# kai422/DAS3R

Hardware: AMD Instinct MI355X
Metric: render fwd+bwd Msplats/s at 1080p (higher is better)
Workload: dtype f32; 1 GPU; 1M random splats, 1920x1080, SH degree 3, forward+backward (BASELINE.json configs[3], constant P); splats_per_gpu=1000000, splats_per_gpu_final=1000000, init_steps=30, sh_degree=3, num_rendered=2614506, api=GaussianRasterizer.forward + autograd backward (drop-in surface), parallelism=1 independent scenes, one per GPU

## Files before the change

das3r_amd/csrc/preprocess.hip:

```cpp
#include "common.h"
#include "granule.h"
#include "segkey.h"
#include "splat_math.h"
#include "pretransform_math.h"

namespace das3r {

template <bool HAS_SH, bool HAS_COV, bool STAGE, bool AA = false>
__global__ void __launch_bounds__(256) preprocess_kernel(
    int P, int D, int M, const float *__restrict__ means3D, const float *__restrict__ scales, float scale_modifier,
    const float *__restrict__ rotations, const float *__restrict__ opacities, const float *__restrict__ shs,
    const float *__restrict__ cov3D_precomp, const float *__restrict__ colors_precomp, const float *__restrict__ viewmatrix,
    const float *__restrict__ projmatrix, const float *__restrict__ campos, int W, int H, float tanfovx, float tanfovy,
    int tiles_x, int tiles_y, int32_t *__restrict__ radii, uint32_t *__restrict__ depth_key, float4 *__restrict__ xyh,
    float4 *__restrict__ conic_opacity, float4 *__restrict__ rgbd, uint8_t *__restrict__ clamped,
    uint32_t *__restrict__ tiles_touched, uint32_t *__restrict__ rect32, int tight_rect , uint32_t *__restrict__ zero_a, uint32_t zero_a_words, uint32_t *__restrict__ zero_b,
    uint32_t zero_b_words, uint32_t *__restrict__ zero_c, uint32_t zero_c_words, unsigned long long *__restrict__ arrive,
    uint32_t *__restrict__ host_out, uint32_t tag, const EmitArgs em,
    uint32_t *__restrict__ dhist ,
    uint32_t dhist_mask ,
    uint32_t *__restrict__ dhist_next ,
    const PreXform pre ,
    float *__restrict__ shjac ) {
    const int gidx = blockIdx.x * blockDim.x + threadIdx.x;
    bool sampled = false;
    if (dhist != nullptr) {
        uint32_t h = blockIdx.x * 0x9E3779B1u;
        h ^= h >> 15; h *= 0x85EBCA6Bu; h ^= h >> 13; h *= 0xC2B2AE35u; h ^= h >> 16;
        sampled = (h & dhist_mask) == 0u;
    }
    const bool live = gidx < P;
    const int idx = live ? gidx : P - 1;
    float3 p, s_in = make_float3(0.f, 0.f, 0.f);
    float op;
    float4 q_in = make_float4(0.f, 0.f, 0.f, 0.f);
    float c3_in[6] = {0.f, 0.f, 0.f, 0.f, 0.f, 0.f};
    if (!HAS_COV && pre.xyz != nullptr) {
        PoseRegs pose;
        load_pose(pre.Rm, pre.tv, pre.Lq, pose);
        const float rx = pre.xyz[3 * idx], ry = pre.xyz[3 * idx + 1], rz = pre.xyz[3 * idx + 2];
        const float4 rq = reinterpret_cast<const float4 *>(pre.rot)[idx];
        const float r0 = pre.scaling[3 * idx], r1 = pre.scaling[3 * idx + 1], r2 = pre.scaling[3 * idx + 2];
        const float ro = pre.opacity_raw[idx];
        const float rc = pre.conf_flat[pre.mask_index ? pre.mask_index[idx] : (int64_t)idx];
        p = pre_mean(pose, rx, ry, rz);
        q_in = pre_rot(pose, rq);
        s_in = make_float3(pre_scale(r0), pre_scale(r1), pre_scale(r2));
        op = pre_opacity(ro, rc);
    } else {
        p = make_float3(means3D[3 * idx], means3D[3 * idx + 1], means3D[3 * idx + 2]);
        op = opacities[idx];
        if (HAS_COV) {
#pragma unroll
            for (int i = 0; i < 6; i++) c3_in[i] = cov3D_precomp[6 * idx + i];
        } else {
            s_in = make_float3(scales[3 * idx], scales[3 * idx + 1], scales[3 * idx + 2]);
            q_in = reinterpret_cast<const float4 *>(rotations)[idx];
        }
    }
    __shared__ uint32_t s_tiles;
    if (threadIdx.x == 0) s_tiles = 0;
    if (!STAGE) __syncthreads();
    for (uint32_t i = gidx; i < zero_a_words; i += gridDim.x * blockDim.x) zero_a[i] = 0u;
    for (uint32_t i = gidx; i < zero_b_words; i += gridDim.x * blockDim.x) zero_b[i] = 0u;
    for (uint32_t i = gidx; i < zero_c_words; i += gridDim.x * blockDim.x) zero_c[i] = 0u;
    if (dhist_next != nullptr && gidx < DBINS) dhist_next[gidx] = 0u;
    __shared__ float4 sh_lds[STAGE ? 256 * 13 : 256 * 5];
    if (STAGE) {
        const float4 *src = reinterpret_cast<const float4 *>(shs) + (size_t)blockIdx.x * 256 * 12;
        const size_t limit = (size_t)P * 12 - (size_t)blockIdx.x * 256 * 12;
        float4 v[12];
#pragma unroll
        for (int i = 0; i < 12; i++) {
            const size_t f = (size_t)(i * 256 + threadIdx.x);
            v[i] = src[f < limit ? f : limit - 1];
        }
#pragma unroll
        for (int i = 0; i < 12; i++) {
            const int f = i * 256 + threadIdx.x;
            sh_lds[(f / 12) * 13 + (f % 12)] = v[i];
        }
        __syncthreads();
    }
    float V[16], PM[16];
#pragma unroll
    for (int i = 0; i < 16; i++) {
        V[i] = viewmatrix[i];
        PM[i] = projmatrix[i];
    }
    const float focal_x = W / (2.0f * tanfovx), focal_y = H / (2.0f * tanfovy);

    int radius_out = 0;
    uint32_t key_out = 0xFFFFFFFFu, tiles_out = 0;
    uint8_t clamp_out = 0;
    float4 xy_out = make_float4(0.f, 0.f, -1e30f, -1e30f);
    float4 co_out = make_float4(0.f, 0.f, 0.f, 0.f);
    float4 rgbd_out = make_float4(0.f, 0.f, 0.f, 0.f);
    float jac_out[9] = {0.f, 0.f, 0.f, 0.f, 0.f, 0.f, 0.f, 0.f, 0.f};
    int bx0 = 0, by0 = 0, bx1 = 0, by1 = 0;

    const float3 p_view = xform43(p, V);
    if (p_view.z > NEAR_PLANE) {
        const float4 p_hom = xform44(p, PM);
        const float p_w = 1.0f / (p_hom.w + 0.0000001f);
        const float ndc_x = p_hom.x * p_w, ndc_y = p_hom.y * p_w;

        float c3[6];
        if (HAS_COV) {
#pragma unroll
            for (int i = 0; i < 6; i++) c3[i] = c3_in[i];
        } else {
            cov3d_from_scale_rot(s_in, scale_modifier, q_in, c3);
        }
        float T[2][3];
        float3 t;
        bool cx, cy;
        ewa_T(p_view, V, focal_x, focal_y, tanfovx, tanfovy, T, t, cx, cy);
        float a, b, c, a0 = 0.f, c0 = 0.f;
        if constexpr (AA) {
            cov2d_undilated(T, c3, a0, b, c0);
            a = a0 + 0.3f;
            c = c0 + 0.3f;
        } else {
            cov2d_from_T(T, c3, a, b, c);
        }
        const float det = a * c - b * b;
        if (det != 0.0f) {
            const float det_inv = 1.f / det;
            const float conA = c * det_inv, conB = -b * det_inv, conC = a * det_inv;
            const float mid = 0.5f * (a + c);
            const float lambda1 = mid + sqrtf(fmaxf(0.1f, mid * mid - det));
            const float lambda2 = mid - sqrtf(fmaxf(0.1f, mid * mid - det));
            const float my_radius = ceilf(3.f * sqrtf(fmaxf(lambda1, lambda2)));
            const float px = ((ndc_x + 1.0f) * W - 1.0f) * 0.5f;
            const float py = ((ndc_y + 1.0f) * H - 1.0f) * 0.5f;
            const int r = (int)my_radius;
            int rminx, rminy, rmaxx, rmaxy;
            tile_rect(px, py, r, tiles_x, tiles_y, rminx, rminy, rmaxx, rmaxy);
            const int area = (rmaxx - rminx) * (rmaxy - rminy);
            if (area != 0) {
                float3 col;
                if (HAS_SH && STAGE) {
                    float sh[48];
                    const int n4 = (3 * (D + 1) * (D + 1) + 3) >> 2;
#pragma unroll
                    for (int i = 0; i < 12; i++) {
                        if (i < n4) {
                            const float4 v = sh_lds[threadIdx.x * 13 + i];
                            sh[4 * i] = v.x; sh[4 * i + 1] = v.y; sh[4 * i + 2] = v.z; sh[4 * i + 3] = v.w;
                        }
                    }
                    col = sh_regs_to_rgb(D, sh, p, campos, clamp_out);
                    if (shjac != nullptr) sh_ddir_regs(D, sh, p, campos, jac_out);
                } else if (HAS_SH) {
                    float sh[48];
                    const float *row = shs + (size_t)idx * M * 3;
                    load_sh_row(row, D, sh_vec_ok(row, D, M), sh);
                    col = sh_regs_to_rgb(D, sh, p, campos, clamp_out);
                    if (shjac != nullptr) sh_ddir_regs(D, sh, p, campos, jac_out);
                } else {
                    col = make_float3(colors_precomp[3 * idx], colors_precomp[3 * idx + 1], colors_precomp[3 * idx + 2]);
                }
                radius_out = r;
                key_out = __float_as_uint(p_view.z);
                if constexpr (AA) op = op * aa_factor(aa_rho(a0, b, c0, det));
                float hx = -1e30f, hy = -1e30f;
                if (255.0f * op > 1.0f) {
                    const float tau2 = 2.0f * __logf(255.0f * op) * 1.0005f + 1e-3f;
                    hx = sqrtf(tau2 * a) * 1.0005f + 0.02f;
                    hy = sqrtf(tau2 * c) * 1.0005f + 0.02f;
                }
                xy_out = make_float4(px, py, hx, hy);
                binned_rect(xy_out, r, tiles_x, tiles_y, (tight_rect & 1) != 0, bx0, by0, bx1, by1);
                tiles_out = (uint32_t)((bx1 - bx0) * (by1 - by0));
                co_out = make_float4(conA, conB, conC, op);
                rgbd_out = make_float4(col.x, col.y, col.z, p_view.z);
            }
        }
    } else if ((tight_rect & 2) && live) {
        __hip_atomic_store(host_out + 12, tag, __ATOMIC_RELAXED, __HIP_MEMORY_SCOPE_SYSTEM);
        __threadfence_system();
    }
    if (live) {
    radii[idx] = radius_out;
    depth_key[idx] = key_out;
    tiles_touched[idx] = tiles_out;
    rect32[idx] = tiles_out ? ((uint32_t)bx0 | ((uint32_t)bx1 << 8) | ((uint32_t)by0 << 16) | ((uint32_t)by1 << 24)) : 0u;
    clamped[idx] = clamp_out;
    if (HAS_SH && shjac != nullptr) {
#pragma unroll
        for (int j = 0; j < 9; j++) shjac[(size_t)j * P + idx] = jac_out[j];
    }
    }
    {
        __syncthreads();
        float4 *rec = sh_lds;
        const int t = threadIdx.x, slot = t * 5;
        rec[slot] = xy_out;
        rec[slot + 1] = co_out;
        rec[slot + 2] = rgbd_out;
        rec[slot + 3] = make_float4(__int_as_float(radius_out), __uint_as_float(tiles_out), 0.f, 0.f);
        __syncthreads();
        float4 *dst = xyh + (size_t)blockIdx.x * 256 * SPLAT_REC;
        const size_t lim = ((size_t)P - (size_t)blockIdx.x * 256) * SPLAT_REC;
#pragma unroll
        for (int i = 0; i < 4; i++) {
            const int f = i * 256 + t;
            if ((size_t)f < lim) dst[f] = rec[f + (f >> 2)];
        }
        if (em.status != nullptr || sampled) __syncthreads();
    }
    if (sampled) {
        uint32_t *lh = reinterpret_cast<uint32_t *>(sh_lds);
        lh[threadIdx.x] = 0u;
        __syncthreads();
        if (live && tiles_out) atomicAdd(&lh[depth_bin(key_out)], tiles_out);
        __syncthreads();
        const uint32_t c = lh[threadIdx.x];
        if (c) atomicAdd(&dhist[threadIdx.x], c);
    }

    if (em.status != nullptr) {
        __shared__ uint32_t ws[4], s_carry;
        uint32_t(*h)[RADIX_SIZE] = reinterpret_cast<uint32_t(*)[RADIX_SIZE]>(sh_lds);
        const int tid = threadIdx.x, lane = __lane_id(), wave = tid >> 6;
        const uint32_t b = blockIdx.x;
        const uint32_t mine = live ? tiles_out : 0u;
        uint32_t total;
        const uint32_t ex = block_exclusive_scan_256(mine, ws, &total);
#pragma unroll
        for (int q = 0; q < 4; q++) h[q][tid] = 0u;
        if (wave == 0) {
            constexpr uint32_t GS = 64u;
            const uint32_t grp = b / GS, r = b % GS, nblocks = gridDim.x;
            const u64 t64 = (u64)em.tag << 32;
            if (lane == 0) granule_store(em.status + b, t64 | total);
            uint32_t in_group = 0, before = 0;
            unsigned spins = 0;
            {
                const bool has = (uint32_t)lane < r;
                u64 x = t64;
                while (true) {
                    if (has) x = granule_poll(em.status + (b - r) + lane, spins);
                    if (__all((x >> 32) == (u64)em.tag)) break;
                    if (spins == SOFT_SPINS && lane == 0) atomicOr(em.err, ERR_HARD_POLL);
                    if (++spins > SPIN_LIMIT) { if (lane == 0) atomicOr(em.err, ERR_TIMEOUT); break; }
                    __builtin_amdgcn_s_sleep(2);
                }
                in_group = has ? (uint32_t)x : 0u;
#pragma unroll
                for (int o = 32; o >= 1; o >>= 1) in_group += (uint32_t)__shfl_xor((int)in_group, o, 64);
            }
            if (r == GS - 1u && lane == 0) granule_store(em.status + nblocks + grp, t64 | (u64)(in_group + total));
            for (uint32_t p0 = 0; p0 < grp; p0 += 64u) {
                const bool has = p0 + (uint32_t)lane < grp;
                u64 x = t64;
                while (true) {
                    if (has) x = granule_poll(em.status + nblocks + p0 + lane, spins);
                    if (__all((x >> 32) == (u64)em.tag)) break;
                    if (spins == SOFT_SPINS && lane == 0) atomicOr(em.err, ERR_HARD_POLL);
                    if (++spins > SPIN_LIMIT) { if (lane == 0) atomicOr(em.err, ERR_TIMEOUT); break; }
                    __builtin_amdgcn_s_sleep(2);
                }
                uint32_t v = has ? (uint32_t)x : 0u;
#pragma unroll
                for (int o = 32; o >= 1; o >>= 1) v += (uint32_t)__shfl_xor((int)v, o, 64);
                before += v;
            }
            if (lane == 0) s_carry = in_group + before;
        }
        __syncthreads();
        uint32_t o = s_carry + ex;
        if (live) {
            em.off_by_gid[idx] = o;
            for (int y = by0; y < by1; y++)
                for (int x = bx0; x < bx1; x++) {
                    if (o < em.cap) {
                        const uint32_t t = (uint32_t)(y * tiles_x + x);
                        em.tile_keys[o] = t;
                        em.gids[o] = (uint32_t)idx;
                        for (int q = 0, sh = 0, dw = tile_digit_width(em.tbits); sh < em.tbits; q++, sh += dw) {
                            const int bits = (em.tbits - sh) < dw ? (em.tbits - sh) : dw;
                            atomicAdd(&h[q][(t >> sh) & ((1u << bits) - 1u)], 1u);
                        }
                    }
                    o++;
                }
        }
        if (b == gridDim.x - 1 && tid == 0) {
            const uint32_t count = s_carry + total, flags = *em.err;
            em.count[0] = count;
            em.count[1] = flags;
            em.count_out[0] = count;
            em.count_out[1] = flags;
            __hip_atomic_store(em.count_out + 2, em.tag, __ATOMIC_RELEASE, __HIP_MEMORY_SCOPE_SYSTEM);
        }
        __syncthreads();
        for (int q = 0, sh = 0, dw = tile_digit_width(em.tbits); sh < em.tbits; q++, sh += dw) {
            const uint32_t c = h[q][tid];
            if (c) atomicAdd(&em.ghist[q * RADIX_SIZE + tid], c);
        }
        return;
    }
    if (arrive == nullptr) return;
    uint32_t wsum = live ? tiles_out : 0u;
#pragma unroll
    for (int o = 32; o >= 1; o >>= 1) wsum += (uint32_t)__shfl_xor((int)wsum, o, 64);
    if (__lane_id() == 0 && wsum) atomicAdd(&s_tiles, wsum);
    __syncthreads();
    if (threadIdx.x == 0) {
        constexpr unsigned long long LOW = (1ull << 40) - 1ull;
        const unsigned r = blockIdx.x & 63u;
        const unsigned long long expected = (gridDim.x - r + 63u) / 64u;
        unsigned long long mine = (1ull << 40) | (unsigned long long)s_tiles;
        unsigned long long *sub = arrive + 8 + 8 * r;
        unsigned long long old = atomicAdd(sub, mine);
        if ((old >> 40) + 1ull == expected) {
            __hip_atomic_store(sub, 0ull, __ATOMIC_RELAXED, __HIP_MEMORY_SCOPE_AGENT);
            mine = (1ull << 40) | ((old + mine) & LOW);
            old = atomicAdd(arrive, mine);
            const unsigned long long subs = gridDim.x < 64u ? gridDim.x : 64u;
            if ((old >> 40) + 1ull == subs) {
                const unsigned long long total = (old + mine) & LOW;
                __hip_atomic_store(arrive, 0ull, __ATOMIC_RELAXED, __HIP_MEMORY_SCOPE_AGENT);
                host_out[0] = (uint32_t)(total > 0xFFFFFFFFull ? 0xFFFFFFFFull : total);
                __hip_atomic_store(host_out + 2, tag, __ATOMIC_RELEASE, __HIP_MEMORY_SCOPE_SYSTEM);
            }
        }
    }
}

__global__ void __launch_bounds__(256) mark_visible_kernel(int P, const float *__restrict__ means3D,
                                                           const float *__restrict__ viewmatrix, uint8_t *__restrict__ present) {
    const int idx = blockIdx.x * blockDim.x + threadIdx.x;
    if (idx >= P) return;
    float V[16];
#pragma unroll
    for (int i = 0; i < 16; i++) V[i] = viewmatrix[i];
    const float3 p = make_float3(means3D[3 * idx], means3D[3 * idx + 1], means3D[3 * idx + 2]);
    present[idx] = xform43(p, V).z > NEAR_PLANE ? 1 : 0;
}

int launch_preprocess(const das3r_raster_args *a, const das3r_raster_in *in, int32_t *radii, char *geom, char *img, char *binning_ctrl,
                      size_t binning_ctrl_bytes, const Layout &L, unsigned long long *arrive, uint32_t *host_out, uint32_t tag,
                      hipStream_t s, const EmitArgs *emit, uint32_t *dhist, uint32_t *dhist_next, bool aa) {
    const int P = a->P;
    if (P == 0) return DAS3R_OK;
    const EmitArgs em = emit ? *emit : EmitArgs{nullptr, 0u, nullptr, nullptr, nullptr, nullptr, nullptr, 0u, 0, nullptr, nullptr};
    dim3 grid(div_up(P, 256)), block(256);
    uint32_t dhist_mask = 0u;
    while ((grid.x >> __builtin_popcount(dhist_mask)) > 512u) dhist_mask = (dhist_mask << 1) | 1u;
    const bool has_sh = in->shs != nullptr, has_cov = in->cov3D_precomp != nullptr;
    const PreXform pre = pre_xform(in);
    float *const shjac = has_sh && L.g_shjac ? (float *)(geom + L.g_shjac) : nullptr;
#define ARGS                                                                                                              \
    P, a->sh_degree, a->M, in->means3D, in->scales, a->scale_modifier, in->rotations, in->opacities, in->shs,             \
        in->cov3D_precomp, in->colors_precomp, a->viewmatrix, a->projmatrix, a->campos, a->image_width, a->image_height,  \
        a->tanfovx, a->tanfovy, L.tiles_x, L.tiles_y, radii, (uint32_t *)(geom + L.g_keyA), (float4 *)(geom + L.pub.xy),  \
        (float4 *)(geom + L.pub.conic_opacity), (float4 *)(geom + L.pub.rgbd), (uint8_t *)(geom + L.pub.clamped),         \
        (uint32_t *)(geom + L.pub.tiles_touched), (uint32_t *)(geom + L.g_rect), (use_tight_rect() ? 1 : 0) | (a->prefiltered ? 2 : 0), (uint32_t *)(geom + L.g_ghist), (uint32_t)(L.g_ctrl_bytes / 4),                 \
        (uint32_t *)(img + L.pub.ranges), (uint32_t)(2 * L.ntiles), (uint32_t *)binning_ctrl, (uint32_t)(binning_ctrl_bytes / 4), arrive, host_out, tag, em, dhist, dhist_mask, dhist_next, pre, shjac
    const bool stage = has_sh && a->M == 16 && a->sh_degree >= 2 && ((uintptr_t)in->shs & 15) == 0 && !switches().no_sh_stage;
#define LAUNCH_PRE(SH, COV, ST)                                                                                   \
    do {                                                                                                          \
        if (aa) DAS3R_LAUNCH((preprocess_kernel<SH, COV, ST, true>), grid, block, 0, s, ARGS);                   \
        else DAS3R_LAUNCH((preprocess_kernel<SH, COV, ST>), grid, block, 0, s, ARGS);                            \
    } while (0)
    if (has_sh && !has_cov && stage) LAUNCH_PRE(true, false, true);
    else if (has_sh && has_cov && stage) LAUNCH_PRE(true, true, true);
    else if (has_sh && !has_cov) LAUNCH_PRE(true, false, false);
    else if (has_sh && has_cov) LAUNCH_PRE(true, true, false);
    else if (!has_sh && !has_cov) LAUNCH_PRE(false, false, false);
    else LAUNCH_PRE(false, true, false);
#undef LAUNCH_PRE
#undef ARGS
    KERNEL_CHECK(s, a->debug, "preprocess");
    return DAS3R_OK;
}

int launch_mark_visible(int P, const float *means3D, const float *viewmatrix, uint8_t *present, hipStream_t s) {
    if (P == 0) return DAS3R_OK;
    DAS3R_LAUNCH(mark_visible_kernel, dim3(div_up(P, 256)), dim3(256), 0, s, P, means3D, viewmatrix, present);
    KERNEL_CHECK(s, false, "mark_visible");
    return DAS3R_OK;
}

}
```

das3r_amd/csrc/splat_math.h:

```cpp
#pragma once
#include <hip/hip_runtime.h>

namespace das3r {

__device__ constexpr float SH_C0 = 0.28209479177387814f;
__device__ constexpr float SH_C1 = 0.4886025119029199f;
__device__ constexpr float SH_C2_0 = 1.0925484305920792f, SH_C2_1 = -1.0925484305920792f, SH_C2_2 = 0.31539156525252005f,
                           SH_C2_3 = -1.0925484305920792f, SH_C2_4 = 0.5462742152960396f;
__device__ constexpr float SH_C3_0 = -0.5900435899266435f, SH_C3_1 = 2.890611442640554f, SH_C3_2 = -0.4570457994644658f,
                           SH_C3_3 = 0.3731763325901154f, SH_C3_4 = -0.4570457994644658f, SH_C3_5 = 1.445305721320277f,
                           SH_C3_6 = -0.5900435899266435f;

__device__ __forceinline__ float3 xform43(const float3 p, const float *m) {
    return make_float3(m[0] * p.x + m[4] * p.y + m[8] * p.z + m[12], m[1] * p.x + m[5] * p.y + m[9] * p.z + m[13],
                       m[2] * p.x + m[6] * p.y + m[10] * p.z + m[14]);
}
__device__ __forceinline__ float4 xform44(const float3 p, const float *m) {
    return make_float4(m[0] * p.x + m[4] * p.y + m[8] * p.z + m[12], m[1] * p.x + m[5] * p.y + m[9] * p.z + m[13],
                       m[2] * p.x + m[6] * p.y + m[10] * p.z + m[14], m[3] * p.x + m[7] * p.y + m[11] * p.z + m[15]);
}

__device__ __forceinline__ void quat_to_R(const float4 q, float R[3][3]) {
    const float r = q.x, x = q.y, y = q.z, z = q.w;
    R[0][0] = 1.f - 2.f * (y * y + z * z); R[0][1] = 2.f * (x * y - r * z);       R[0][2] = 2.f * (x * z + r * y);
    R[1][0] = 2.f * (x * y + r * z);       R[1][1] = 1.f - 2.f * (x * x + z * z); R[1][2] = 2.f * (y * z - r * x);
    R[2][0] = 2.f * (x * z - r * y);       R[2][1] = 2.f * (y * z + r * x);       R[2][2] = 1.f - 2.f * (x * x + y * y);
}

__device__ __forceinline__ void cov3d_from_scale_rot(const float3 scale, const float mod, const float4 q, float *cov) {
    float R[3][3];
    quat_to_R(q, R);
    const float s[3] = {mod * scale.x, mod * scale.y, mod * scale.z};
    float Mm[3][3];
#pragma unroll
    for (int i = 0; i < 3; i++)
#pragma unroll
        for (int k = 0; k < 3; k++) Mm[i][k] = R[i][k] * s[k];
#define SIG(i, j) (Mm[i][0] * Mm[j][0] + Mm[i][1] * Mm[j][1] + Mm[i][2] * Mm[j][2])
    cov[0] = SIG(0, 0); cov[1] = SIG(0, 1); cov[2] = SIG(0, 2); cov[3] = SIG(1, 1); cov[4] = SIG(1, 2); cov[5] = SIG(2, 2);
#undef SIG
}

__device__ __forceinline__ void ewa_T(const float3 p_view, const float *V, const float focal_x, const float focal_y,
                                      const float tanfovx, const float tanfovy, float T[2][3], float3 &t, bool &clampx, bool &clampy) {
    t = p_view;
    const float limx = 1.3f * tanfovx, limy = 1.3f * tanfovy;
    const float txtz = t.x / t.z, tytz = t.y / t.z;
    clampx = (txtz < -limx || txtz > limx);
    clampy = (tytz < -limy || tytz > limy);
    t.x = fminf(limx, fmaxf(-limx, txtz)) * t.z;
    t.y = fminf(limy, fmaxf(-limy, tytz)) * t.z;
    const float J00 = focal_x / t.z, J02 = -(focal_x * t.x) / (t.z * t.z);
    const float J11 = focal_y / t.z, J12 = -(focal_y * t.y) / (t.z * t.z);
#pragma unroll
    for (int j = 0; j < 3; j++) {
        T[0][j] = J00 * V[4 * j + 0] + 0.f * V[4 * j + 1] + J02 * V[4 * j + 2];
        T[1][j] = 0.f * V[4 * j + 0] + J11 * V[4 * j + 1] + J12 * V[4 * j + 2];
    }
}

__device__ __forceinline__ void cov2d_undilated(const float T[2][3], const float *c3, float &a0, float &b, float &c0) {
    const float S[3][3] = {{c3[0], c3[1], c3[2]}, {c3[1], c3[3], c3[4]}, {c3[2], c3[4], c3[5]}};
    float TS[2][3];
#pragma unroll
    for (int i = 0; i < 2; i++)
#pragma unroll
        for (int j = 0; j < 3; j++) TS[i][j] = T[i][0] * S[0][j] + T[i][1] * S[1][j] + T[i][2] * S[2][j];
    a0 = TS[0][0] * T[0][0] + TS[0][1] * T[0][1] + TS[0][2] * T[0][2];
    b = TS[0][0] * T[1][0] + TS[0][1] * T[1][1] + TS[0][2] * T[1][2];
    c0 = TS[1][0] * T[1][0] + TS[1][1] * T[1][1] + TS[1][2] * T[1][2];
}

__device__ __forceinline__ void cov2d_from_T(const float T[2][3], const float *c3, float &a, float &b, float &c) {
    float a0, c0;
    cov2d_undilated(T, c3, a0, b, c0);
    a = a0 + 0.3f;
    c = c0 + 0.3f;
}

constexpr float AA_RHO_MIN = 2.5e-5f;
__device__ __forceinline__ float aa_rho(const float a0, const float b, const float c0, const float det) { return (a0 * c0 - b * b) / det; }
__device__ __forceinline__ float aa_factor(const float rho) { return sqrtf(fmaxf(rho, AA_RHO_MIN)); }

__device__ __forceinline__ void tile_rect(const float px, const float py, const int r, const int tiles_x, const int tiles_y,
                                          int &rminx, int &rminy, int &rmaxx, int &rmaxy) {
    rminx = min(tiles_x, max(0, (int)((px - r) / TILE_X)));
    rminy = min(tiles_y, max(0, (int)((py - r) / TILE_Y)));
    rmaxx = min(tiles_x, max(0, (int)((px + r + TILE_X - 1) / TILE_X)));
    rmaxy = min(tiles_y, max(0, (int)((py + r + TILE_Y - 1) / TILE_Y)));
}

__device__ __forceinline__ void binned_rect(const float4 xyh, const int r, const int tiles_x, const int tiles_y, const bool tight,
                                            int &rminx, int &rminy, int &rmaxx, int &rmaxy) {
    tile_rect(xyh.x, xyh.y, r, tiles_x, tiles_y, rminx, rminy, rmaxx, rmaxy);
    if (tight) {
        if (xyh.z < 0.f) {
            rmaxx = rminx;
            return;
        }
        const float px0 = ceilf(xyh.x - xyh.z), px1 = floorf(xyh.x + xyh.z);
        const float py0 = ceilf(xyh.y - xyh.w), py1 = floorf(xyh.y + xyh.w);
        if (px1 < px0 || py1 < py0 || px1 < 0.f || py1 < 0.f) {
            rmaxx = rminx;
            return;
        }
        const int tx0 = (int)fmaxf(px0, 0.f) >> 4, ty0 = (int)fmaxf(py0, 0.f) >> 4;
        const int tx1 = ((int)fminf(px1, 1.0e6f) >> 4) + 1, ty1 = ((int)fminf(py1, 1.0e6f) >> 4) + 1;
        rminx = max(rminx, tx0);
        rminy = max(rminy, ty0);
        rmaxx = max(rminx, min(rmaxx, tx1));
        rmaxy = max(rminy, min(rmaxy, ty1));
    }
}

__device__ __forceinline__ void load_sh_row(const float *__restrict__ row, const int D, const bool vec_ok, float sh[48]) {
    const int n3 = 3 * (D + 1) * (D + 1);
    if (vec_ok) {
        const float4 *r4 = reinterpret_cast<const float4 *>(row);
#pragma unroll
        for (int i = 0; i < 12; i++) {
            if (4 * i < n3) {
                const float4 v = r4[i];
                sh[4 * i] = v.x; sh[4 * i + 1] = v.y; sh[4 * i + 2] = v.z; sh[4 * i + 3] = v.w;
            }
        }
    } else {
#pragma unroll
        for (int i = 0; i < 48; i++)
            if (i < n3) sh[i] = row[i];
    }
}

__device__ __forceinline__ float3 sh_eval(const int deg, const float sh[48], const float x, const float y, const float z) {
    float out[3];
#pragma unroll
    for (int c = 0; c < 3; c++) {
#define SHC(k) sh[(k) * 3 + c]
        float r = SH_C0 * SHC(0);
        if (deg > 0) {
            r = r - SH_C1 * y * SHC(1) + SH_C1 * z * SHC(2) - SH_C1 * x * SHC(3);
            if (deg > 1) {
                const float xx = x * x, yy = y * y, zz = z * z, xy = x * y, yz = y * z, xz = x * z;
                r = r + SH_C2_0 * xy * SHC(4) + SH_C2_1 * yz * SHC(5) + SH_C2_2 * (2.f * zz - xx - yy) * SHC(6) +
                    SH_C2_3 * xz * SHC(7) + SH_C2_4 * (xx - yy) * SHC(8);
                if (deg > 2) {
                    r = r + SH_C3_0 * y * (3.f * xx - yy) * SHC(9) + SH_C3_1 * xy * z * SHC(10) +
                        SH_C3_2 * y * (4.f * zz - xx - yy) * SHC(11) + SH_C3_3 * z * (2.f * zz - 3.f * xx - 3.f * yy) * SHC(12) +
                        SH_C3_4 * x * (4.f * zz - xx - yy) * SHC(13) + SH_C3_5 * z * (xx - yy) * SHC(14) +
                        SH_C3_6 * x * (xx - 3.f * yy) * SHC(15);
                }
            }
        }
#undef SHC
        out[c] = r + 0.5f;
    }
    return make_float3(out[0], out[1], out[2]);
}

#define SH_DDIR(SHC, dRdx, dRdy, dRdz)                                                                                          \
    do {                                                                                                                        \
        dRdx = 0.f; dRdy = 0.f; dRdz = 0.f;                                                                                     \
        if (D > 0) {                                                                                                            \
            dRdx = -SH_C1 * SHC(3);                                                                                             \
            dRdy = -SH_C1 * SHC(1);                                                                                             \
            dRdz = SH_C1 * SHC(2);                                                                                              \
            if (D > 1) {                                                                                                        \
                dRdx += SH_C2_0 * y * SHC(4) + SH_C2_2 * 2.f * -x * SHC(6) + SH_C2_3 * z * SHC(7) + SH_C2_4 * 2.f * x * SHC(8); \
                dRdy += SH_C2_0 * x * SHC(4) + SH_C2_1 * z * SHC(5) + SH_C2_2 * 2.f * -y * SHC(6) + SH_C2_4 * 2.f * -y * SHC(8); \
                dRdz += SH_C2_1 * y * SHC(5) + SH_C2_2 * 2.f * 2.f * z * SHC(6) + SH_C2_3 * x * SHC(7);                       \
                if (D > 2) {                                                                                                    \
                    dRdx += SH_C3_0 * SHC(9) * 3.f * 2.f * xy + SH_C3_1 * SHC(10) * yz + SH_C3_2 * SHC(11) * -2.f * xy +       \
                            SH_C3_3 * SHC(12) * -3.f * 2.f * xz + SH_C3_4 * SHC(13) * (-3.f * xx + 4.f * zz - yy) +            \
                            SH_C3_5 * SHC(14) * 2.f * xz + SH_C3_6 * SHC(15) * 3.f * (xx - yy);                                \
                    dRdy += SH_C3_0 * SHC(9) * 3.f * (xx - yy) + SH_C3_1 * SHC(10) * xz +                                      \
                            SH_C3_2 * SHC(11) * (-3.f * yy + 4.f * zz - xx) + SH_C3_3 * SHC(12) * -3.f * 2.f * yz +            \
                            SH_C3_4 * SHC(13) * -2.f * xy + SH_C3_5 * SHC(14) * -2.f * yz + SH_C3_6 * SHC(15) * -3.f * 2.f * xy; \
                    dRdz += SH_C3_1 * SHC(10) * xy + SH_C3_2 * SHC(11) * 4.f * 2.f * yz +                                      \
                            SH_C3_3 * SHC(12) * 3.f * (2.f * zz - xx - yy) + SH_C3_4 * SHC(13) * 4.f * 2.f * xz +              \
                            SH_C3_5 * SHC(14) * (xx - yy);                                                                      \
                }                                                                                                               \
            }                                                                                                                   \
        }                                                                                                                       \
    } while (0)

__device__ __forceinline__ bool sh_vec_ok(const float *row, const int D, const int M) {
    const int n3 = 3 * (D + 1) * (D + 1);
    return (((uintptr_t)row & 15) == 0) && (((n3 + 3) & ~3) <= 3 * M);
}

__device__ __forceinline__ float3 sh_regs_to_rgb(const int D, const float sh[48], const float3 p, const float *campos,
                                                 uint8_t &clamp_bits) {
    const float dx = p.x - campos[0], dy = p.y - campos[1], dz = p.z - campos[2];
    const float inv = 1.f / sqrtf(dx * dx + dy * dy + dz * dz);
    const float3 r = sh_eval(D, sh, dx * inv, dy * inv, dz * inv);
    clamp_bits = (uint8_t)((r.x < 0.f ? 1 : 0) | (r.y < 0.f ? 2 : 0) | (r.z < 0.f ? 4 : 0));
    return make_float3(fmaxf(r.x, 0.f), fmaxf(r.y, 0.f), fmaxf(r.z, 0.f));
}

__device__ __forceinline__ void sh_ddir_regs(const int D, const float sh[48], const float3 p, const float *campos, float J[9]) {
    const float dx = p.x - campos[0], dy = p.y - campos[1], dz = p.z - campos[2];
    const float inv = 1.f / sqrtf(dx * dx + dy * dy + dz * dz);
    const float x = dx * inv, y = dy * inv, z = dz * inv;
    const float xx = x * x, yy = y * y, zz = z * z, xy = x * y, yz = y * z, xz = x * z;
#pragma unroll
    for (int c = 0; c < 3; c++) {
#define SHC_REG(k) sh[(k) * 3 + c]
        SH_DDIR(SHC_REG, J[3 * c], J[3 * c + 1], J[3 * c + 2]);
#undef SHC_REG
    }
}

}
```

Measured before the change: 1143 Msplats/s.

## Split SH staging into two LDS phases to shrink shared memory and raise occupancy

The staged preprocess kernel now stages spherical-harmonic coefficients through shared memory in two halves: the first 7 float4s per splat are evaluated first, then the remaining 5 are written into the same LDS buffer and evaluated. This cuts LDS from 13 to 7 float4 per thread, and a min-waves launch bound is added so more blocks can be resident per CU. In exchange, the high-half coefficients are held in registers across the low-half evaluation, and the kernel gains extra block-wide barriers. The added launch bound may also force register spilling.

```diff
diff --git a/das3r_amd/csrc/preprocess.hip b/das3r_amd/csrc/preprocess.hip
--- a/das3r_amd/csrc/preprocess.hip
+++ b/das3r_amd/csrc/preprocess.hip
@@ -6,8 +6,11 @@
 
 namespace das3r {
 
+typedef float v4f __attribute__((ext_vector_type(4)));
+constexpr int STAGE_WAVES = 5;
+
 template <bool HAS_SH, bool HAS_COV, bool STAGE, bool AA = false>
-__global__ void __launch_bounds__(256) preprocess_kernel(
+__global__ void __launch_bounds__(256, STAGE ? STAGE_WAVES : 1) preprocess_kernel(
     int P, int D, int M, const float *__restrict__ means3D, const float *__restrict__ scales, float scale_modifier,
     const float *__restrict__ rotations, const float *__restrict__ opacities, const float *__restrict__ shs,
     const float *__restrict__ cov3D_precomp, const float *__restrict__ colors_precomp, const float *__restrict__ viewmatrix,
@@ -65,21 +68,27 @@
     for (uint32_t i = gidx; i < zero_b_words; i += gridDim.x * blockDim.x) zero_b[i] = 0u;
     for (uint32_t i = gidx; i < zero_c_words; i += gridDim.x * blockDim.x) zero_c[i] = 0u;
     if (dhist_next != nullptr && gidx < DBINS) dhist_next[gidx] = 0u;
-    __shared__ float4 sh_lds[STAGE ? 256 * 13 : 256 * 5];
+    __shared__ float4 sh_lds[STAGE ? 256 * 7 : 256 * 5];
+    v4f sh_hi[STAGE ? 5 : 1];
     if (STAGE) {
-        const float4 *src = reinterpret_cast<const float4 *>(shs) + (size_t)blockIdx.x * 256 * 12;
+        const v4f *src = reinterpret_cast<const v4f *>(shs) + (size_t)blockIdx.x * 256 * 12;
         const size_t limit = (size_t)P * 12 - (size_t)blockIdx.x * 256 * 12;
-        float4 v[12];
-#pragma unroll
-        for (int i = 0; i < 12; i++) {
-            const size_t f = (size_t)(i * 256 + threadIdx.x);
-            v[i] = src[f < limit ? f : limit - 1];
-        }
-#pragma unroll
-        for (int i = 0; i < 12; i++) {
-            const int f = i * 256 + threadIdx.x;
-            sh_lds[(f / 12) * 13 + (f % 12)] = v[i];
-        }
+        v4f sh_lo[7];
+#pragma unroll
+        for (int i = 0; i < 7; i++) {
+            const int j = i * 256 + threadIdx.x;
+            const size_t f = (size_t)((j / 7) * 12 + j % 7);
+            sh_lo[i] = src[f < limit ? f : limit - 1];
+        }
+#pragma unroll
+        for (int i = 0; i < 5; i++) {
+            const int j = i * 256 + threadIdx.x;
+            const size_t f = (size_t)((j / 5) * 12 + 7 + j % 5);
+            sh_hi[i] = src[f < limit ? f : limit - 1];
+        }
+#pragma unroll
+        for (int i = 0; i < 7; i++)
+            reinterpret_cast<v4f *>(sh_lds)[i * 256 + threadIdx.x] = sh_lo[i];
         __syncthreads();
     }
     float V[16], PM[16];
@@ -98,6 +107,7 @@
     float4 rgbd_out = make_float4(0.f, 0.f, 0.f, 0.f);
     float jac_out[9] = {0.f, 0.f, 0.f, 0.f, 0.f, 0.f, 0.f, 0.f, 0.f};
     int bx0 = 0, by0 = 0, bx1 = 0, by1 = 0;
+    bool shade = false;
 
     const float3 p_view = xform43(p, V);
     if (p_view.z > NEAR_PLANE) {
@@ -139,19 +149,9 @@
             tile_rect(px, py, r, tiles_x, tiles_y, rminx, rminy, rmaxx, rmaxy);
             const int area = (rmaxx - rminx) * (rmaxy - rminy);
             if (area != 0) {
-                float3 col;
+                float3 col = make_float3(0.f, 0.f, 0.f);
                 if (HAS_SH && STAGE) {
-                    float sh[48];
-                    const int n4 = (3 * (D + 1) * (D + 1) + 3) >> 2;
-#pragma unroll
-                    for (int i = 0; i < 12; i++) {
-                        if (i < n4) {
-                            const float4 v = sh_lds[threadIdx.x * 13 + i];
-                            sh[4 * i] = v.x; sh[4 * i + 1] = v.y; sh[4 * i + 2] = v.z; sh[4 * i + 3] = v.w;
-                        }
-                    }
-                    col = sh_regs_to_rgb(D, sh, p, campos, clamp_out);
-                    if (shjac != nullptr) sh_ddir_regs(D, sh, p, campos, jac_out);
+                    shade = true;
                 } else if (HAS_SH) {
                     float sh[48];
                     const float *row = shs + (size_t)idx * M * 3;
@@ -180,6 +180,58 @@
     } else if ((tight_rect & 2) && live) {
         __hip_atomic_store(host_out + 12, tag, __ATOMIC_RELAXED, __HIP_MEMORY_SCOPE_SYSTEM);
         __threadfence_system();
+    }
+    if (STAGE) {
+        float sh[48], col_acc[3];
+        float3 dir = make_float3(0.f, 0.f, 0.f);
+        if (shade) {
+            const float dx = p.x - campos[0], dy = p.y - campos[1], dz = p.z - campos[2];
+            const float inv = 1.f / sqrtf(dx * dx + dy * dy + dz * dz);
+            dir = make_float3(dx * inv, dy * inv, dz * inv);
+#pragma unroll
+            for (int i = 0; i < 7; i++) {
+                const float4 v = sh_lds[threadIdx.x * 7 + i];
+                sh[4 * i] = v.x; sh[4 * i + 1] = v.y; sh[4 * i + 2] = v.z; sh[4 * i + 3] = v.w;
+            }
+            const float x = dir.x, y = dir.y, z = dir.z;
+            const float xx = x * x, yy = y * y, zz = z * z, xy = x * y, yz = y * z, xz = x * z;
+#pragma unroll
+            for (int c = 0; c < 3; c++) {
+#define SHC_ROW(k) sh[(k) * 3 + c]
+                SH_EVAL_LO(SHC_ROW, col_acc[c]);
+                if (shjac != nullptr) SH_DDIR_LO(SHC_ROW, jac_out[3 * c], jac_out[3 * c + 1], jac_out[3 * c + 2]);
+#undef SHC_ROW
+            }
+        }
+        if (D > 2) {
+            __syncthreads();
+#pragma unroll
+            for (int i = 0; i < 5; i++) reinterpret_cast<v4f *>(sh_lds)[i * 256 + threadIdx.x] = sh_hi[i];
+            __syncthreads();
+            if (shade) {
+#pragma unroll
+                for (int i = 0; i < 5; i++) {
+                    const float4 v = sh_lds[threadIdx.x * 5 + i];
+                    sh[28 + 4 * i] = v.x; sh[29 + 4 * i] = v.y; sh[30 + 4 * i] = v.z; sh[31 + 4 * i] = v.w;
+                }
+                const float x = dir.x, y = dir.y, z = dir.z;
+                const float xx = x * x, yy = y * y, zz = z * z, xy = x * y, yz = y * z, xz = x * z;
+#pragma unroll
+                for (int c = 0; c < 3; c++) {
+#define SHC_ROW(k) sh[(k) * 3 + c]
+                    SH_EVAL_HI(SHC_ROW, col_acc[c]);
+                    if (shjac != nullptr) SH_DDIR_HI(SHC_ROW, jac_out[3 * c], jac_out[3 * c + 1], jac_out[3 * c + 2]);
+#undef SHC_ROW
+                }
+            }
+        }
+        if (shade) {
+            const float r0 = col_acc[0] + 0.5f, r1 = col_acc[1] + 0.5f, r2 = col_acc[2] + 0.5f;
+            clamp_out = (uint8_t)((r0 < 0.f ? 1 : 0) | (r1 < 0.f ? 2 : 0) | (r2 < 0.f ? 4 : 0));
+            rgbd_out.x = fmaxf(r0, 0.f);
+            rgbd_out.y = fmaxf(r1, 0.f);
+            rgbd_out.z = fmaxf(r2, 0.f);
+        }
     }
     if (live) {
     radii[idx] = radius_out;
diff --git a/das3r_amd/csrc/splat_math.h b/das3r_amd/csrc/splat_math.h
--- a/das3r_amd/csrc/splat_math.h
+++ b/das3r_amd/csrc/splat_math.h
@@ -183,6 +183,42 @@
         }                                                                                                                       \
     } while (0)
 
+#define SH_EVAL_LO(SHC, r)                                                                                                      \
+    do {                                                                                                                        \
+        r = SH_C0 * SHC(0);                                                                                                     \
+        r = r - SH_C1 * y * SHC(1) + SH_C1 * z * SHC(2) - SH_C1 * x * SHC(3);                                                   \
+        r = r + SH_C2_0 * xy * SHC(4) + SH_C2_1 * yz * SHC(5) + SH_C2_2 * (2.f * zz - xx - yy) * SHC(6) +                       \
+            SH_C2_3 * xz * SHC(7) + SH_C2_4 * (xx - yy) * SHC(8);                                                               \
+    } while (0)
+#define SH_EVAL_HI(SHC, r)                                                                                                      \
+    do {                                                                                                                        \
+        r = r + SH_C3_0 * y * (3.f * xx - yy) * SHC(9) + SH_C3_1 * xy * z * SHC(10) +                                           \
+            SH_C3_2 * y * (4.f * zz - xx - yy) * SHC(11) + SH_C3_3 * z * (2.f * zz - 3.f * xx - 3.f * yy) * SHC(12) +           \
+            SH_C3_4 * x * (4.f * zz - xx - yy) * SHC(13) + SH_C3_5 * z * (xx - yy) * SHC(14) +                                  \
+            SH_C3_6 * x * (xx - 3.f * yy) * SHC(15);                                                                            \
+    } while (0)
+#define SH_DDIR_LO(SHC, dRdx, dRdy, dRdz)                                                                                       \
+    do {                                                                                                                        \
+        dRdx = -SH_C1 * SHC(3);                                                                                                 \
+        dRdy = -SH_C1 * SHC(1);                                                                                                 \
+        dRdz = SH_C1 * SHC(2);                                                                                                  \
+        dRdx += SH_C2_0 * y * SHC(4) + SH_C2_2 * 2.f * -x * SHC(6) + SH_C2_3 * z * SHC(7) + SH_C2_4 * 2.f * x * SHC(8);         \
+        dRdy += SH_C2_0 * x * SHC(4) + SH_C2_1 * z * SHC(5) + SH_C2_2 * 2.f * -y * SHC(6) + SH_C2_4 * 2.f * -y * SHC(8);        \
+        dRdz += SH_C2_1 * y * SHC(5) + SH_C2_2 * 2.f * 2.f * z * SHC(6) + SH_C2_3 * x * SHC(7);                                 \
+    } while (0)
+#define SH_DDIR_HI(SHC, dRdx, dRdy, dRdz)                                                                                       \
+    do {                                                                                                                        \
+        dRdx += SH_C3_0 * SHC(9) * 3.f * 2.f * xy + SH_C3_1 * SHC(10) * yz + SH_C3_2 * SHC(11) * -2.f * xy +                   \
+                SH_C3_3 * SHC(12) * -3.f * 2.f * xz + SH_C3_4 * SHC(13) * (-3.f * xx + 4.f * zz - yy) +                        \
+                SH_C3_5 * SHC(14) * 2.f * xz + SH_C3_6 * SHC(15) * 3.f * (xx - yy);                                            \
+        dRdy += SH_C3_0 * SHC(9) * 3.f * (xx - yy) + SH_C3_1 * SHC(10) * xz +                                                  \
+                SH_C3_2 * SHC(11) * (-3.f * yy + 4.f * zz - xx) + SH_C3_3 * SHC(12) * -3.f * 2.f * yz +                        \
+                SH_C3_4 * SHC(13) * -2.f * xy + SH_C3_5 * SHC(14) * -2.f * yz + SH_C3_6 * SHC(15) * -3.f * 2.f * xy;           \
+        dRdz += SH_C3_1 * SHC(10) * xy + SH_C3_2 * SHC(11) * 4.f * 2.f * yz +                                                  \
+                SH_C3_3 * SHC(12) * 3.f * (2.f * zz - xx - yy) + SH_C3_4 * SHC(13) * 4.f * 2.f * xz +                          \
+                SH_C3_5 * SHC(14) * (xx - yy);                                                                                  \
+    } while (0)
+
 __device__ __forceinline__ bool sh_vec_ok(const float *row, const int D, const int M) {
     const int n3 = 3 * (D + 1) * (D + 1);
     return (((uintptr_t)row & 15) == 0) && (((n3 + 3) & ~3) <= 3 * M);
```

New measurement: 1147 Msplats/s (median of 6 runs). About the same (+0.3%).
